# broadinstitute/Tangram

Hardware: NVIDIA H100
Metric: map_cells_to_space iterations/sec (higher is better)
Workload: dtype bf16 operands / f32 accumulate+state

## Files before the change

tangram_b200/csrc/gemm_tc.cuh:

```cuda
#pragma once
#include <cuda.h>
#include <cstdio>
#include "common.cuh"
#include "gemm_simt.cuh"

namespace tgb {

constexpr int TC_BM = 128;
constexpr int TC_BK = 64;
constexpr int TC_MMA_K = 16;
constexpr int TC_BN = 256;
constexpr int TC_THREADS = 384;
constexpr int TC_ACC = TC_BN / 2;

__device__ __forceinline__ uint32_t smem_u32(const void* p) { return (uint32_t)__cvta_generic_to_shared(p); }

__device__ __forceinline__ void mbar_init(uint64_t* bar, uint32_t count) {
  asm volatile("mbarrier.init.shared::cta.b64 [%0], %1;" ::"r"(smem_u32(bar)), "r"(count));
}
__device__ __forceinline__ void mbar_expect_tx(uint64_t* bar, uint32_t bytes) {
  asm volatile("mbarrier.arrive.expect_tx.shared::cta.b64 _, [%0], %1;" ::"r"(smem_u32(bar)), "r"(bytes) : "memory");
}
__device__ __forceinline__ void mbar_wait(uint64_t* bar, uint32_t parity) {
  asm volatile(
// ... 27 lines not shown
constexpr uint64_t kPolicyEvictLast = 0x14F0000000000000ull;
constexpr uint64_t kPolicyEvictFirst = 0x12F0000000000000ull;
__device__ __forceinline__ void prefetch_l2(const void* p) { asm volatile("prefetch.global.L2 [%0];" ::"l"(p)); }
__device__ __forceinline__ void tma_load_2d(const CUtensorMap* map, uint64_t* bar, void* dst, int c0, int c1, uint64_t policy) {
  asm volatile(
      "cp.async.bulk.tensor.2d.shared::cluster.global.tile.mbarrier::complete_tx::bytes.L2::cache_hint [%0], [%1, {%3, %4}], [%2], %5;"
      ::"r"(smem_u32(dst)), "l"(map), "r"(smem_u32(bar)), "r"(c0), "r"(c1), "l"(policy) : "memory");
}
__device__ __forceinline__ void tma_load_2d_pair(const CUtensorMap* map, uint64_t* bar, void* dst, int c0, int c1, uint64_t policy) {
  asm volatile(
      "cp.async.bulk.tensor.2d.shared::cluster.global.tile.mbarrier::complete_tx::bytes.multicast::cluster.L2::cache_hint"
      " [%0], [%1, {%3, %4}], [%2], %5, %6;"
      ::"r"(smem_u32(dst)), "l"(map), "r"(smem_u32(bar)), "r"(c0), "r"(c1), "h"((uint16_t)0x3), "l"(policy) : "memory");
}
__device__ __forceinline__ void tma_prefetch_desc(const CUtensorMap* map) {
  asm volatile("prefetch.tensormap [%0];" ::"l"(map) : "memory");
}
__device__ __forceinline__ void tma_store_2d(const CUtensorMap* map, const void* src, int c0, int c1, uint64_t policy) {
  asm volatile(
      "cp.async.bulk.tensor.2d.global.shared::cta.bulk_group.L2::cache_hint [%0, {%2, %3}], [%1], %4;"
      ::"l"(map), "r"(smem_u32(src)), "r"(c0), "r"(c1), "l"(policy) : "memory");
}
__device__ __forceinline__ void bulk_commit() { asm volatile("cp.async.bulk.commit_group;" ::: "memory"); }
__device__ __forceinline__ void bulk_wait_read_all() { asm volatile("cp.async.bulk.wait_group.read 0;" ::: "memory"); }
__device__ __forceinline__ void fence_proxy_async_smem() { asm volatile("fence.proxy.async.shared::cta;" ::: "memory"); }
template <int ID>
__device__ __forceinline__ void named_bar_sync(int threads) {
  asm volatile("bar.sync %0, %1;" ::"n"(ID), "r"(threads) : "memory");
}
__device__ __forceinline__ void ldmatrix_x4(uint32_t addr, uint32_t (&r)[4]) {
  asm volatile("ldmatrix.sync.aligned.m8n8.x4.shared.b16 {%0, %1, %2, %3}, [%4];"
               : "=r"(r[0]), "=r"(r[1]), "=r"(r[2]), "=r"(r[3]) : "r"(addr) : "memory");
}
__device__ __forceinline__ void stmatrix_x4(uint32_t addr, const uint32_t (&r)[4]) {
  asm volatile("stmatrix.sync.aligned.m8n8.x4.shared.b16 [%0], {%1, %2, %3, %4};"
               ::"r"(addr), "r"(r[0]), "r"(r[1]), "r"(r[2]), "r"(r[3]) : "memory");
}

__device__ __forceinline__ void setmaxnreg_producer() { asm volatile("setmaxnreg.dec.sync.aligned.u32 40;"); }
__device__ __forceinline__ void setmaxnreg_consumer() { asm volatile("setmaxnreg.inc.sync.aligned.u32 232;"); }

__device__ __forceinline__ void wgmma_fence() { asm volatile("wgmma.fence.sync.aligned;" ::: "memory"); }
__device__ __forceinline__ void wgmma_commit() { asm volatile("wgmma.commit_group.sync.aligned;" ::: "memory"); }
template <int N>
__device__ __forceinline__ void wgmma_wait() { asm volatile("wgmma.wait_group.sync.aligned %0;" ::"n"(N) : "memory"); }
__device__ __forceinline__ void acc_fence(float (&d)[TC_ACC]) {
#pragma unroll
  for (int i = 0; i < TC_ACC; ++i) asm volatile("" : "+f"(d[i])::"memory");
}

template <int TA, int TB>
__device__ __forceinline__ void wgmma_m64n256k16(float (&d)[128], uint64_t a_desc, uint64_t b_desc, uint32_t accumulate) {
  asm volatile(
      "{\n\t.reg .pred p;\n\t"
      "setp.ne.b32 p, %130, 0;\n\t"
      "wgmma.mma_async.sync.aligned.m64n256k16.f32.bf16.bf16 {"
      "%0,%1,%2,%3,%4,%5,%6,%7,%8,%9,%10,%11,%12,%13,%14,%15,"
      "%16,%17,%18,%19,%20,%21,%22,%23,%24,%25,%26,%27,%28,%29,%30,%31,"
      "%32,%33,%34,%35,%36,%37,%38,%39,%40,%41,%42,%43,%44,%45,%46,%47,"
      "%48,%49,%50,%51,%52,%53,%54,%55,%56,%57,%58,%59,%60,%61,%62,%63,"
      "%64,%65,%66,%67,%68,%69,%70,%71,%72,%73,%74,%75,%76,%77,%78,%79,"
      "%80,%81,%82,%83,%84,%85,%86,%87,%88,%89,%90,%91,%92,%93,%94,%95,"
      "%96,%97,%98,%99,%100,%101,%102,%103,%104,%105,%106,%107,%108,%109,%110,%111,"
      "%112,%113,%114,%115,%116,%117,%118,%119,%120,%121,%122,%123,%124,%125,%126,%127"
      "}, %128, %129, p, 1, 1, %131, %132;\n\t}"
      : "+f"(d[0]), "+f"(d[1]), "+f"(d[2]), "+f"(d[3]), "+f"(d[4]), "+f"(d[5]), "+f"(d[6]), "+f"(d[7]),
        "+f"(d[8]), "+f"(d[9]), "+f"(d[10]), "+f"(d[11]), "+f"(d[12]), "+f"(d[13]), "+f"(d[14]), "+f"(d[15]),
        "+f"(d[16]), "+f"(d[17]), "+f"(d[18]), "+f"(d[19]), "+f"(d[20]), "+f"(d[21]), "+f"(d[22]), "+f"(d[23]),
        "+f"(d[24]), "+f"(d[25]), "+f"(d[26]), "+f"(d[27]), "+f"(d[28]), "+f"(d[29]), "+f"(d[30]), "+f"(d[31]),
        "+f"(d[32]), "+f"(d[33]), "+f"(d[34]), "+f"(d[35]), "+f"(d[36]), "+f"(d[37]), "+f"(d[38]), "+f"(d[39]),
        "+f"(d[40]), "+f"(d[41]), "+f"(d[42]), "+f"(d[43]), "+f"(d[44]), "+f"(d[45]), "+f"(d[46]), "+f"(d[47]),
        "+f"(d[48]), "+f"(d[49]), "+f"(d[50]), "+f"(d[51]), "+f"(d[52]), "+f"(d[53]), "+f"(d[54]), "+f"(d[55]),
        "+f"(d[56]), "+f"(d[57]), "+f"(d[58]), "+f"(d[59]), "+f"(d[60]), "+f"(d[61]), "+f"(d[62]), "+f"(d[63]),
        "+f"(d[64]), "+f"(d[65]), "+f"(d[66]), "+f"(d[67]), "+f"(d[68]), "+f"(d[69]), "+f"(d[70]), "+f"(d[71]),
        "+f"(d[72]), "+f"(d[73]), "+f"(d[74]), "+f"(d[75]), "+f"(d[76]), "+f"(d[77]), "+f"(d[78]), "+f"(d[79]),
        "+f"(d[80]), "+f"(d[81]), "+f"(d[82]), "+f"(d[83]), "+f"(d[84]), "+f"(d[85]), "+f"(d[86]), "+f"(d[87]),
        "+f"(d[88]), "+f"(d[89]), "+f"(d[90]), "+f"(d[91]), "+f"(d[92]), "+f"(d[93]), "+f"(d[94]), "+f"(d[95]),
        "+f"(d[96]), "+f"(d[97]), "+f"(d[98]), "+f"(d[99]), "+f"(d[100]), "+f"(d[101]), "+f"(d[102]), "+f"(d[103]),
        "+f"(d[104]), "+f"(d[105]), "+f"(d[106]), "+f"(d[107]), "+f"(d[108]), "+f"(d[109]), "+f"(d[110]), "+f"(d[111]),
        "+f"(d[112]), "+f"(d[113]), "+f"(d[114]), "+f"(d[115]), "+f"(d[116]), "+f"(d[117]), "+f"(d[118]), "+f"(d[119]),
        "+f"(d[120]), "+f"(d[121]), "+f"(d[122]), "+f"(d[123]), "+f"(d[124]), "+f"(d[125]), "+f"(d[126]), "+f"(d[127])
      : "l"(a_desc), "l"(b_desc), "r"(accumulate), "n"(TA), "n"(TB));
}
__device__ __forceinline__ uint64_t make_smem_desc(uint32_t saddr, uint32_t lbo_bytes, uint32_t sbo_bytes) {
  uint64_t d = 0;
  d |= (uint64_t)((saddr & 0x3FFFF) >> 4);
  d |= (uint64_t)((lbo_bytes >> 4) & 0x3FFF) << 16;
  d |= (uint64_t)((sbo_bytes >> 4) & 0x3FFF) << 32;
  d |= (uint64_t)1 << 62;
  return d;
}

template <bool KMAJOR, int ROWS>
struct OperandTile {
  static constexpr int kBytes = ROWS * TC_BK * 2;
  static __device__ __forceinline__ void load(const CUtensorMap* map, uint64_t* bar, uint8_t* dst, int mn0, int k0, uint64_t policy) {
    if (KMAJOR) {
      tma_load_2d(map, bar, dst, k0, mn0, policy);
    } else {
#pragma unroll
      for (int b = 0; b < ROWS / 64; ++b) tma_load_2d(map, bar, dst + b * 8192, mn0 + b * 64, k0, policy);
    }
  }
  static __device__ __forceinline__ void load_half_pair(const CUtensorMap* map, uint64_t* bar, uint8_t* dst, int mn0, int k0, int h,
                                                        uint64_t policy) {
    constexpr int HALF = ROWS / 2;
    if (KMAJOR) {
      tma_load_2d_pair(map, bar, dst + h * HALF * 128, k0, mn0 + h * HALF, policy);
    } else {
#pragma unroll
      for (int b = 0; b < HALF / 64; ++b)
        tma_load_2d_pair(map, bar, dst + h * HALF * 128 + b * 8192, mn0 + h * HALF + b * 64, k0, policy);
    }
  }
  static __device__ __forceinline__ uint64_t desc(uint32_t saddr, int k_step ) {
    if (KMAJOR) return make_smem_desc(saddr + k_step * (TC_MMA_K * 2), 16, 1024);
    return make_smem_desc(saddr + k_step * (TC_MMA_K * 128), 8192, 1024);
  }
};

struct EpiSmem {
  uint8_t* buf;
  uint64_t* full;
  uint64_t* free;
  uint32_t parity;
};
__device__ __forceinline__ void tile_mn(int w, int tiles_m, int tiles_n, int group_m, int& m, int& n) {
  const int per_group = group_m * tiles_n;
  const int g = w / per_group, r = w - g * per_group;
  const int rows = min(group_m, tiles_m - g * group_m);
  n = r / rows;
  m = g * group_m + (r - n * rows);
}
struct TileCoord {
  int m0, n0;
  int tile_n;
  int tiles_n;
  int split;
};

__device__ __forceinline__ float quad_sum(float v) {
  v += __shfl_xor_sync(0xffffffffu, v, 1);
  v += __shfl_xor_sync(0xffffffffu, v, 2);
  return v;
}

struct TcEpiStore {
  static constexpr int kSmemBytes = 0;
  float* C; int ldc; size_t split_stride; int M;
  int accumulate;
  __device__ __forceinline__ void prologue(const TileCoord&, int) const {}
  __device__ __forceinline__ void load(int, int, const EpiSmem&) const {}
  __device__ __forceinline__ void run(const float (&d)[TC_ACC], const TileCoord& t, int row, int lane, int, const EpiSmem&) const {
    float* base = C + (size_t)t.split * split_stride;
#pragma unroll
    for (int h = 0; h < 2; ++h) {
      const int r = row + 8 * h;
      if (r >= M) continue;
#pragma unroll
      for (int j = 0; j < TC_BN / 8; ++j) {
        const int col = t.n0 + 8 * j + 2 * (lane & 3);
        if (col < ldc) {
          float2* dst = reinterpret_cast<float2*>(base + (size_t)r * ldc + col);
          float2 v = make_float2(d[4 * j + 2 * h], d[4 * j + 2 * h + 1]);
          if (accumulate) { const float2 o = *dst; v.x += o.x; v.y += o.y; }
          *dst = v;
        }
      }
    }
  }
};

struct TcEpiDpStore {
  static constexpr int kSmemBytes = TC_BM * TC_BN * 2;
  static constexpr int kHalfBytes = kSmemBytes / 2;
  static constexpr int kBoxBytes = 64 * 128;
  CUtensorMap pt_map, dq_map;
  int ld;
  const float* center;
  float* rpart;
  int M;
  __device__ __forceinline__ int boxes(int r0, int n0) const { return r0 < M ? min(TC_BN / 64, (ld - n0) / 64) : 0; }
  __device__ __forceinline__ void prologue(const TileCoord&, int) const {}
  __device__ __forceinline__ void load(int m0, int n0, const EpiSmem& es) const {
#pragma unroll
    for (int h = 0; h < 2; ++h) {
      mbar_wait(&es.free[h], es.parity ^ 1);
      const int nb = boxes(m0 + 64 * h, n0);
      mbar_expect_tx(&es.full[h], nb * kBoxBytes);
      for (int b = 0; b < nb; ++b)
        tma_load_2d(&pt_map, &es.full[h], es.buf + h * kHalfBytes + b * kBoxBytes, n0 + 64 * b, m0 + 64 * h, kPolicyEvictFirst);
    }
  }
  __device__ __forceinline__ void run(const float (&d)[TC_ACC], const TileCoord& t, int row, int lane, int cw,
                                      const EpiSmem& es) const {
    const int r0 = t.m0 + 64 * cw;
    const int nb = boxes(r0, t.n0);
    float c[2];
#pragma unroll
    for (int h = 0; h < 2; ++h) c[h] = row + 8 * h < M ? center[row + 8 * h] : 0.f;
    const int mi = lane >> 3, rr = lane & 7;
    const int arow = ((row - r0) & ~15) + 8 * (mi & 1) + rr;
    const uint32_t half = smem_u32(es.buf + cw * kHalfBytes) + arow * 128;
    mbar_wait(&es.full[cw], es.parity);
    float racc[2] = {0.f, 0.f};
#pragma unroll
    for (int b = 0; b < TC_BN / 64; ++b) {
      if (b >= nb) break;
#pragma unroll
      for (int q = 0; q < 4; ++q) {
        const uint32_t addr = half + b * kBoxBytes + (((2 * q + (mi >> 1)) ^ rr) << 4);
        uint32_t p[4], o[4];
        ldmatrix_x4(addr, p);
#pragma unroll
        for (int e = 0; e < 2; ++e) {
          const int j = 8 * b + 2 * q + e;
#pragma unroll
          for (int h = 0; h < 2; ++h) {
            const __nv_bfloat162 d2 = __floats2bfloat162_rn(d[4 * j + 2 * h] - c[h], d[4 * j + 2 * h + 1] - c[h]);
            const __nv_bfloat162 p2 = *reinterpret_cast<const __nv_bfloat162*>(&p[2 * e + h]);
            racc[h] = fmaf(__low2float(p2), __low2float(d2), racc[h]);
            racc[h] = fmaf(__high2float(p2), __high2float(d2), racc[h]);
            o[2 * e + h] = *reinterpret_cast<const uint32_t*>(&d2);
          }
        }
        stmatrix_x4(addr, o);
      }
    }
    fence_proxy_async_smem();
    if (cw == 0) named_bar_sync<1>(128); else named_bar_sync<2>(128);
    if ((threadIdx.x & 127) == 0) {
      for (int b = 0; b < nb; ++b) tma_store_2d(&dq_map, es.buf + cw * kHalfBytes + b * kBoxBytes, t.n0 + 64 * b, r0, kPolicyEvictFirst);
      bulk_commit();
      bulk_wait_read_all();
      mbar_arrive(&es.free[cw]);
    }
#pragma unroll
    for (int h = 0; h < 2; ++h) {
      const float s = quad_sum(racc[h]);
      if (row + 8 * h < M && (lane & 3) == 0) rpart[(size_t)t.tile_n * M + row + 8 * h] = s;
    }
  }
};

struct TcEpiDpStoreF32 {
  static constexpr int kSmemBytes = 0;
  float* dp; int ld;
  const __nv_bfloat16* P3; size_t plane;
  float* rpart;
  int M;
  __device__ __forceinline__ void prologue(const TileCoord& t, int ct) const {
#pragma unroll
    for (int i = ct; i < 3 * TC_BM * (TC_BN / 64); i += 256) {
      const int pl = i / (TC_BM * (TC_BN / 64)), li = i - pl * (TC_BM * (TC_BN / 64));
      const int row = t.m0 + (li >> 2), col = t.n0 + (li & 3) * 64;
      if (row < M && col < ld) prefetch_l2(P3 + pl * plane + (size_t)row * ld + col);
    }
  }
  __device__ __forceinline__ void load(int, int, const EpiSmem&) const {}
  __device__ __forceinline__ void run(const float (&d)[TC_ACC], const TileCoord& t, int row, int lane, int, const EpiSmem&) const {
#pragma unroll
    for (int h = 0; h < 2; ++h) {
      const int r = row + 8 * h;
      const bool live = r < M;
      const __nv_bfloat16* prow = P3 + (size_t)r * ld;
      float* drow = dp + (size_t)r * ld;
      float racc = 0.f;
#pragma unroll
      for (int j = 0; j < TC_BN / 8; ++j) {
        const int col = t.n0 + 8 * j + 2 * (lane & 3);
        if (live && col < ld) {
          const __nv_bfloat162 h2 = *reinterpret_cast<const __nv_bfloat162*>(prow + col);
          const __nv_bfloat162 m2 = *reinterpret_cast<const __nv_bfloat162*>(prow + plane + col);
          const __nv_bfloat162 l2 = *reinterpret_cast<const __nv_bfloat162*>(prow + 2 * plane + col);
          const float p0 = (__low2float(l2) + __low2float(m2)) + __low2float(h2);
          const float p1 = (__high2float(l2) + __high2float(m2)) + __high2float(h2);
          const float v0 = d[4 * j + 2 * h], v1 = d[4 * j + 2 * h + 1];
          racc = fmaf(p0, v0, racc);
          racc = fmaf(p1, v1, racc);
          *reinterpret_cast<float2*>(drow + col) = make_float2(v0, v1);
        }
      }
      racc = quad_sum(racc);
      if (live && (lane & 3) == 0) rpart[(size_t)t.tile_n * M + r] = racc;
    }
  }
};

struct __align__(16) RowConst { float lse, r, h, pad; };

__device__ __forceinline__ float fast_ex2(float x) { float y; asm("ex2.approx.ftz.f32 %0, %1;" : "=f"(y) : "f"(x)); return y; }
__device__ __forceinline__ float fast_rcp(float x) { float y; asm("rcp.approx.ftz.f32 %0, %1;" : "=f"(y) : "f"(x)); return y; }
__device__ __forceinline__ float fast_sqrt(float x) { float y; asm("sqrt.approx.ftz.f32 %0, %1;" : "=f"(y) : "f"(x)); return y; }

struct TcMaps { CUtensorMap m[3]; };
__device__ __constant__ int kPairA[6] = {2, 0, 1, 1, 0, 0};
__device__ __constant__ int kPairB[6] = {0, 2, 1, 0, 1, 0};

template <bool A_KMAJOR, bool B_KMAJOR, int STAGES, class Epi>
__global__ void __launch_bounds__(TC_THREADS, 1)
k_gemm_tc(const __grid_constant__ TcMaps maps_a, const __grid_constant__ TcMaps maps_b, int n_pairs,
          int k_total, int k_per_split, int tiles_m, int tiles_n, int splits, int group_m, uint64_t policy_a,
          uint64_t policy_b, int tm_off, int k_off, const __grid_constant__ Epi epi) {
  using TileA = OperandTile<A_KMAJOR, TC_BM>;
  using TileB = OperandTile<B_KMAJOR, TC_BN>;
  constexpr int kStageBytes = TileA::kBytes + TileB::kBytes;
  constexpr int kTA = A_KMAJOR ? 0 : 1, kTB = B_KMAJOR ? 0 : 1;
  constexpr uint32_t kConsumerWarps = 8;

  extern __shared__ uint8_t smem_raw[];
  uint8_t* smem = reinterpret_cast<uint8_t*>(((uintptr_t)smem_raw + 1023) & ~(uintptr_t)1023);
  __shared__ __align__(8) uint64_t full_bar[STAGES];
  __shared__ __align__(8) uint64_t empty_bar[STAGES];
  __shared__ __align__(8) uint64_t epi_full[2], epi_free[2];

  const int wg = threadIdx.x >> 7, lane = threadIdx.x & 31;
  const int tiles_mp = (tiles_m + 1) / 2;
  const int total = tiles_mp * tiles_n * splits;
  EpiSmem es{smem + STAGES * kStageBytes, epi_full, epi_free, 0};

  if (threadIdx.x == 0) {
    tma_prefetch_desc(&maps_a.m[0]);
    tma_prefetch_desc(&maps_b.m[0]);
#pragma unroll
    for (int s = 0; s < STAGES; ++s) { mbar_init(&full_bar[s], 1); mbar_init(&empty_bar[s], 2 * kConsumerWarps); }
    if constexpr (Epi::kSmemBytes > 0) {
      for (int h = 0; h < 2; ++h) { mbar_init(&epi_full[h], 1); mbar_init(&epi_free[h], 1); }
    }
    fence_barrier_init();
  }
  cluster_sync();

  if (wg == 0) {
    setmaxnreg_producer();
    if (threadIdx.x == 0) {
      uint32_t kbg = 0;
      for (int w = cluster_index(); w < total; w += cluster_count()) {
        const int z = w / (tiles_n * tiles_mp);
        int tp_i, tn_i;
        tile_mn(w - z * tiles_n * tiles_mp, tiles_mp, tiles_n, group_m, tp_i, tn_i);
        const int tm_i = 2 * tp_i + cluster_rank();
        const bool live = tm_i < tiles_m;
        const int n0 = tn_i * TC_BN, m0 = (tm_off + tm_i) * TC_BM;
        const int k_begin = k_off + z * k_per_split;
        const int k_end = min(k_total, k_begin + k_per_split);
        const int num_kb = (k_end - k_begin + TC_BK - 1) / TC_BK;
        for (int pr = 6 - n_pairs; pr < 6; ++pr) {
          const CUtensorMap* ma = &maps_a.m[kPairA[pr]];
          const CUtensorMap* mb = &maps_b.m[kPairB[pr]];
#pragma unroll 1
          for (int kb = 0; kb < num_kb; ++kb, ++kbg) {
            const int s = kbg % STAGES;
            const uint32_t ph = (kbg / STAGES) & 1;
            mbar_wait(&empty_bar[s], ph ^ 1);
            uint8_t* sa = smem + s * kStageBytes;
            uint8_t* sb = sa + TileA::kBytes;
            mbar_expect_tx(&full_bar[s], live ? kStageBytes : TileB::kBytes);
            const int k0 = k_begin + kb * TC_BK;
            if (live) TileA::load(ma, &full_bar[s], sa, m0, k0, policy_a);
            TileB::load_half_pair(mb, &full_bar[s], sb, n0, k0, cluster_rank(), policy_b);
#ifndef TGB_SKIP_EPI
            if (Epi::kSmemBytes > 0 && live && pr == 6 - n_pairs && kb + 1 == min(STAGES, num_kb)) epi.load(m0, n0, es);
#endif
          }
        }
        if (live) es.parity ^= 1;
      }
    }
  } else {
    setmaxnreg_consumer();
    const int cw = wg - 1;
    const int ct = threadIdx.x - 128;
    const int row_in_tile = 64 * cw + 16 * ((threadIdx.x >> 5) & 3) + (lane >> 2);
    float acc[TC_ACC];
#pragma unroll
    for (int i = 0; i < TC_ACC; ++i) acc[i] = 0.f;
    uint32_t kbg = 0;
    for (int w = cluster_index(); w < total; w += cluster_count()) {
      TileCoord t;
      t.split = w / (tiles_n * tiles_mp);
      int tp_i;
      tile_mn(w - t.split * tiles_n * tiles_mp, tiles_mp, tiles_n, group_m, tp_i, t.tile_n);
      t.tiles_n = tiles_n;
      t.n0 = t.tile_n * TC_BN;
      t.m0 = (tm_off + 2 * tp_i + cluster_rank()) * TC_BM;
      const bool live = t.m0 < (tm_off + tiles_m) * TC_BM;
      const int k_begin = k_off + t.split * k_per_split;
      const int k_end = min(k_total, k_begin + k_per_split);
      const int total_kb = (k_end - k_begin + TC_BK - 1) / TC_BK * n_pairs;
#ifndef TGB_SKIP_EPI
      if (live) epi.prologue(t, ct);
#endif
      acc_fence(acc);
      for (int kb = 0; kb < total_kb; ++kb, ++kbg) {
        const int s = kbg % STAGES;
        const uint32_t ph = (kbg / STAGES) & 1;
        mbar_wait(&full_bar[s], ph);
        const uint32_t sa = smem_u32(smem + s * kStageBytes) + cw * 8192;
        const uint32_t sb = smem_u32(smem + s * kStageBytes) + TileA::kBytes;
        wgmma_fence();
#pragma unroll
        for (int k = 0; k < TC_BK / TC_MMA_K; ++k)
          wgmma_m64n256k16<kTA, kTB>(acc, TileA::desc(sa, k), TileB::desc(sb, k), (kb > 0 || k > 0) ? 1u : 0u);
        wgmma_commit();
        wgmma_wait<1>();
        if (kb > 0 && lane < 2) mbar_arrive_cluster(&empty_bar[(kbg - 1) % STAGES], lane);
      }
      wgmma_wait<0>();
      acc_fence(acc);
      if (total_kb > 0 && lane < 2) mbar_arrive_cluster(&empty_bar[(kbg - 1) % STAGES], lane);
#ifndef TGB_SKIP_EPI
      if (t.m0 < (tm_off + tiles_m) * TC_BM) {
        epi.run(acc, t, t.m0 + row_in_tile, lane, cw, es);
        es.parity ^= 1;
      }
#endif
    }
  }
  cluster_sync();
}

typedef CUresult (*PFN_encodeTiled)(CUtensorMap*, CUtensorMapDataType, cuuint32_t, void*, const cuuint64_t*,
                                    const cuuint64_t*, const cuuint32_t*, const cuuint32_t*, CUtensorMapInterleave,
                                    CUtensorMapSwizzle, CUtensorMapL2promotion, CUtensorMapFloatOOBfill);

struct TcContext {
  PFN_encodeTiled encode = nullptr;
  int num_sms = 132;
  const void* smem_fn[16] = {};
  int smem_bytes[16] = {};
  int clusters[16] = {};
};

static inline int tc_init(TcContext& tc, char* err, size_t n) {
  void* fn = nullptr;
  cudaDriverEntryPointQueryResult qres;
  cudaError_t e = cudaGetDriverEntryPoint("cuTensorMapEncodeTiled", &fn, cudaEnableDefault, &qres);
  if (e != cudaSuccess || fn == nullptr || qres != cudaDriverEntryPointSuccess) {
    snprintf(err, n, "cuTensorMapEncodeTiled not available from the driver (%s)", cudaGetErrorString(e));
    return -2;
  }
  tc.encode = (PFN_encodeTiled)fn;
  int dev = 0;
  cudaGetDevice(&dev);
  cudaDeviceGetAttribute(&tc.num_sms, cudaDevAttrMultiProcessorCount, dev);
  return 0;
}

static inline int tc_make_map(TcContext& tc, CUtensorMap* map, const void* base, uint64_t cols, uint64_t rows,
                              uint64_t ld, uint32_t box_inner, uint32_t box_outer, char* err, size_t n) {
// ... 153 lines not shown
```

tangram_b200/csrc/tangram_b200.cu:

```cuda
#include "../../include/tangram_b200.h"

#include <algorithm>
#include <cmath>
#include <cstdarg>
#include <cstdio>
#include <cstdlib>
#include <cstring>
#include <mutex>
#include <string>
#include <thread>
#include <vector>

#include "common.cuh"
#include "kernels_elem.cuh"
#include "gemm_simt.cuh"
#include "gemm_tc.cuh"
#include "adam_rows.cuh"
#include "legacy_rng.cuh"
#include "agreement.cuh"
#include "annotate.cuh"
#include "project.cuh"
#include "group_stats.cuh"
#include "neighbors.cuh"
#include "mt19937_jump.h"
// ... 2718 lines not shown
  }
  int bad_host = 0;
  CK(cudaMemcpyAsync(&bad_host, bad.p, sizeof(int), cudaMemcpyDeviceToHost, s));
  CK(cudaStreamSynchronize(s));
  if (bad_host)
    return fail(TGB200_ERR_INVALID, "a CSR column index is outside [0, %lld) or not strictly increasing within its row",
                (long long)n_genes);
  CK(cudaMemcpyAsync(sum_out, sum.p, sizeof(double) * T * G, cudaMemcpyDefault, s));
  CK(cudaMemcpyAsync(sumsq_out, sq.p, sizeof(double) * T * G, cudaMemcpyDefault, s));
  if (nnz_out) CK(cudaMemcpyAsync(nnz_out, cntd.p, sizeof(int64_t) * T * G, cudaMemcpyDefault, s));
  CK(cudaStreamSynchronize(s));
  return TGB200_OK;
}

extern "C" int tgb200_group_stats(const float* X, int64_t x_ld, const int64_t* indptr, const int32_t* indices,
                                  const float* data, int64_t nnz, int64_t rows, int64_t n_genes,
                                  const int32_t* labels, int32_t n_labels, double* sum_out, double* sumsq_out,
                                  int64_t* nnz_out, int64_t block_rows, int32_t device, void* stream) {
  return group_stats_pass(GsValue::kIdentity, 1.0, X, x_ld, indptr, indices, data, nnz, rows, n_genes, labels, n_labels,
                          sum_out, sumsq_out, nnz_out, block_rows, device, stream);
}

extern "C" int tgb200_group_stats_expm1(const float* X, int64_t x_ld, const int64_t* indptr, const int32_t* indices,
                                        const float* data, int64_t nnz, int64_t rows, int64_t n_genes,
                                        const int32_t* labels, int32_t n_labels, double* sum_out, double* sumsq_out,
                                        int64_t* nnz_out, int64_t block_rows, int32_t device, void* stream,
                                        double scale) {
  if (!std::isfinite(scale)) return fail(TGB200_ERR_INVALID, "scale=%g is not finite", scale);
  return group_stats_pass(GsValue::kExpm1, scale, X, x_ld, indptr, indices, data, nnz, rows, n_genes, labels, n_labels,
                          sum_out, sumsq_out, nnz_out, block_rows, device, stream);
}

#ifdef TGB_OVERLAP_PROBE
extern "C" TGB200_API int tgb200_debug_overlap_probe(tgb200_mapper* h, int32_t kind, int32_t cap, int32_t update_ctas,
                                                     int32_t what, int32_t reps, float* out) {
  if (!h || !out || reps < 1 || what < 1 || what > 3) return fail(TGB200_ERR_INVALID, "bad argument");
  if (!h->bf16 || !h->pipelined || h->host_state || !h->plan_dp.ready || !h->plan_fwd.ready)
    return fail(TGB200_ERR_STATE, "needs a resident, pipelined bf16 handle that has run an iteration");
  CK(cudaSetDevice(h->cfg.device));
  const int c0 = h->chunk_row[0], c1 = h->chunk_row[1], c2 = h->chunk_row[2];
  const AdamScalars a = adam_scalars(h->cfg, h->step > 0 ? h->step : 1, 0.1f);
  const AdamRowsArgs ar{h->M.p, h->mb.p, h->v.p, h->dq.p, h->Pb.p, reinterpret_cast<const RowConst*>(h->rowc.p),
                        h->zsum.p, h->pxsum.p, h->l1sum.p, h->l2sum.p, h->ld, h->V, c0, c1,
                        h->cfg.lambda_r, h->cfg.lambda_l1, h->cfg.lambda_l2, a};
  const bool plain = ar.lam_r == 0.f && ar.lam_l1 == 0.f && ar.lam_l2 == 0.f;
  const int keep = cap > 0 ? std::max(0, h->tc.num_sms - 2 * cap) : 0;
  cudaEvent_t ev[4];
  for (auto& e : ev) CK(cudaEventCreate(&e));
  int st = TGB200_OK;
  CK(cudaDeviceSynchronize());
  for (int r = 0; r < reps && st == TGB200_OK; ++r) {
    CK(cudaEventRecord(ev[0], h->hi));
    CK(cudaStreamWaitEvent(h->lo, ev[0], 0));
    if (what & 1) {
      if (kind == 0) {
        TcEpiDpStore epi{h->plan_dp.pt, h->plan_dp.dq, h->ld, h->rcenter.p, h->rpart.p, h->N};
        st = tc_dpstore_launch(h->tc, h->plan_dp, 1, epi, c1, c2, h->V, h->Ke, keep, h->hi, g_err, sizeof(g_err));
      } else {
        st = tc_forward_launch_rows(h->tc, h->plan_fwd, 1, h->Y.p, 1, c1, c2, h->V, h->Ke, keep, h->hi, g_err, sizeof(g_err));
      }
    }
    if (what & 2) {
      if (update_ctas <= 0) {
        if (adam_rows_launch(ar, h->lo)) st = fail(TGB200_ERR_CUDA, "launch adam_rows");
      } else if (plain) {
        k_adam_rows_probe<true><<<update_ctas, 512, 0, h->lo>>>(ar);
      } else {
        k_adam_rows_probe<false><<<update_ctas, 512, 0, h->lo>>>(ar);
      }
      if (cudaGetLastError() != cudaSuccess) st = fail(TGB200_ERR_CUDA, "launch adam_rows_probe");
    }
    CK(cudaEventRecord(ev[1], h->hi));
    CK(cudaEventRecord(ev[2], h->lo));
    CK(cudaStreamWaitEvent(h->hi, ev[2], 0));
    CK(cudaEventRecord(ev[3], h->hi));
    CK(cudaEventSynchronize(ev[3]));
    for (int i = 0; i < 3; ++i) CK(cudaEventElapsedTime(&out[3 * r + i], ev[0], ev[i + 1]));
  }
  for (auto& e : ev) cudaEventDestroy(e);
  return st;
}
#endif

namespace {
constexpr int64_t kNbMaxCellsPerAxis = int64_t(1) << 24;
constexpr int64_t kNbMaxCells = int64_t(1) << 28;

int64_t nb_cell_cap(int64_t n) { return std::min<int64_t>(2 * n + 64, kNbMaxCells); }

nb::Grid nb_grid(const double lo[3], const double ext[3], int64_t n, double per_cell, double min_h, int64_t cap) {
  double log_vol = 0.0, max_ext = 0.0;
  int d_eff = 0;
  for (int a = 0; a < 3; ++a) {
    if (ext[a] > 0) { log_vol += std::log(ext[a]); ++d_eff; }
    max_ext = std::max(max_ext, ext[a]);
  }
  double h = d_eff ? std::exp((log_vol + std::log(per_cell / (double)n)) / d_eff) : 1.0;
  h = std::max(h, min_h);
  if (!(h > 0) || !std::isfinite(1.0 / h)) h = max_ext > 0 ? max_ext : 1.0;
  nb::Grid g{};
  for (;;) {
    const double inv = 1.0 / h;
    double total = 1.0;
    bool ok = true;
    for (int a = 0; a < 3; ++a) {
      const double c = std::floor(ext[a] * inv) + 1.0;
      ok &= c <= (double)kNbMaxCellsPerAxis;
      total *= c;
    }
    if (ok && total <= (double)cap) {
      g.inv_h = inv;
      for (int a = 0; a < 3; ++a) { g.lo[a] = lo[a]; g.nc[a] = (int)(std::floor(ext[a] * inv) + 1.0); }
      break;
    }
    h *= 1.25;
  }
  g.h_lo = (1.0 / g.inv_h) * (1.0 - 1e-9);
  if (!(g.h_lo > 1e-150)) g.h_lo = 0.0;
  return g;
}

struct NbSearch {
  DevBuf<double> C, xs, ys, zs;
  DevBuf<int> orig, cell, count, bad;
  DevBuf<long long> start, tiles;
  DevBuf<unsigned long long> box;
  nb::Grid g{};
  int n = 0;
  nb::Points points() const { return nb::Points{xs.p, ys.p, zs.p, orig.p, start.p}; }
};

int64_t nb_scan_tiles(int64_t n) { return ceil_div(n, nb::kScanTile); }

int nb_scan(const int* in, int64_t n, long long* out, long long* tiles, cudaStream_t s) {
  const int64_t nt = nb_scan_tiles(n);
  nb::k_nb_scan_tiles<<<(unsigned)nt, 256, 0, s>>>(in, n, out, tiles);
  CK(cudaGetLastError());
  lrng::k_scan_counts<<<1, 1024, 0, s>>>(tiles, (int)nt, tiles + nt + 1);
  CK(cudaGetLastError());
  nb::k_nb_scan_add<<<(unsigned)ceil_div(n + 1, nb::kThreads), nb::kThreads, 0, s>>>(out, n, tiles + nt + 1, (int)nt);
  CK(cudaGetLastError());
  return TGB200_OK;
}

double nb_search_bytes(int64_t n, int dim) {
  const int64_t cells = nb_cell_cap(n);
  return 8.0 * n * dim + 32.0 * n + 4.0 * n + 12.0 * (cells + 1) + 16.0 * (nb_scan_tiles(std::max(cells, n) + 1) + 1);
}

int nb_build(const double* coords, int64_t n, int dim, double per_cell, double min_h, double out_bytes, int32_t device,
             cudaStream_t s, const char* what, NbSearch& S) {
  int n_sms = 0;
  CKS(use_sm90_device(device, &n_sms));
  size_t free_b = 0, total_b = 0;
  CK(cudaMemGetInfo(&free_b, &total_b));
  const double need = nb_search_bytes(n, dim) + out_bytes, avail = (double)free_b - 256.0 * (1 << 20);
  if (need > avail)
    return fail(TGB200_ERR_INVALID, "%s over %lld points in %d-D needs %.3f GiB on device %d (%.3f GiB of it for the "
                "output); %.3f GiB are free", what, (long long)n, dim, need / 1073741824.0, device,
                out_bytes / 1073741824.0, free_b / 1073741824.0);
  S.n = (int)n;
  CKS(S.C.alloc((size_t)n * dim, false));
  CK(cudaMemcpyAsync(S.C.p, coords, sizeof(double) * n * dim, cudaMemcpyDefault, s));
  unsigned long long box0[6];
  for (int a = 0; a < 3; ++a) { box0[2 * a] = ~0ull; box0[2 * a + 1] = 0ull; }
  CKS(S.box.alloc(6, false));
// ... 118 lines not shown
```

Measured before the change: 48.08.

## Defer dP-store epilogue into next tile's mainloop to overlap with wgmma

The DpStore epilogue becomes deferred. Each consumer packs its accumulator into bf16 registers and spreads the ldmatrix/stmatrix, TMA store and row-reduction work for the previous tile across specific k-blocks of the next tile's mainloop. The P-tile smem buffer is halved and loaded in two rounds by the producer at chosen k-blocks. A first-MMA variant that zeroes the accumulator replaces explicit accumulator reuse. An optional compile-time phase probe is also added. This aims to hide the epilogue latency behind tensor-core work, at the cost of extra registers (64 packed words) and more complex barrier/parity bookkeeping.

```diff
diff --git a/tangram_b200/csrc/gemm_tc.cuh b/tangram_b200/csrc/gemm_tc.cuh
--- a/tangram_b200/csrc/gemm_tc.cuh
+++ b/tangram_b200/csrc/gemm_tc.cuh
@@ -133,6 +133,39 @@
         "+f"(d[120]), "+f"(d[121]), "+f"(d[122]), "+f"(d[123]), "+f"(d[124]), "+f"(d[125]), "+f"(d[126]), "+f"(d[127])
       : "l"(a_desc), "l"(b_desc), "r"(accumulate), "n"(TA), "n"(TB));
 }
+template <int TA, int TB>
+__device__ __forceinline__ void wgmma_m64n256k16_first(float (&d)[128], uint64_t a_desc, uint64_t b_desc) {
+  asm volatile(
+      "{\n\t.reg .pred p;\n\t"
+      "setp.ne.b32 p, 0, 0;\n\t"
+      "wgmma.mma_async.sync.aligned.m64n256k16.f32.bf16.bf16 {"
+      "%0,%1,%2,%3,%4,%5,%6,%7,%8,%9,%10,%11,%12,%13,%14,%15,"
+      "%16,%17,%18,%19,%20,%21,%22,%23,%24,%25,%26,%27,%28,%29,%30,%31,"
+      "%32,%33,%34,%35,%36,%37,%38,%39,%40,%41,%42,%43,%44,%45,%46,%47,"
+      "%48,%49,%50,%51,%52,%53,%54,%55,%56,%57,%58,%59,%60,%61,%62,%63,"
+      "%64,%65,%66,%67,%68,%69,%70,%71,%72,%73,%74,%75,%76,%77,%78,%79,"
+      "%80,%81,%82,%83,%84,%85,%86,%87,%88,%89,%90,%91,%92,%93,%94,%95,"
+      "%96,%97,%98,%99,%100,%101,%102,%103,%104,%105,%106,%107,%108,%109,%110,%111,"
+      "%112,%113,%114,%115,%116,%117,%118,%119,%120,%121,%122,%123,%124,%125,%126,%127"
+      "}, %128, %129, p, 1, 1, %130, %131;\n\t}"
+      : "=f"(d[0]), "=f"(d[1]), "=f"(d[2]), "=f"(d[3]), "=f"(d[4]), "=f"(d[5]), "=f"(d[6]), "=f"(d[7]),
+        "=f"(d[8]), "=f"(d[9]), "=f"(d[10]), "=f"(d[11]), "=f"(d[12]), "=f"(d[13]), "=f"(d[14]), "=f"(d[15]),
+        "=f"(d[16]), "=f"(d[17]), "=f"(d[18]), "=f"(d[19]), "=f"(d[20]), "=f"(d[21]), "=f"(d[22]), "=f"(d[23]),
+        "=f"(d[24]), "=f"(d[25]), "=f"(d[26]), "=f"(d[27]), "=f"(d[28]), "=f"(d[29]), "=f"(d[30]), "=f"(d[31]),
+        "=f"(d[32]), "=f"(d[33]), "=f"(d[34]), "=f"(d[35]), "=f"(d[36]), "=f"(d[37]), "=f"(d[38]), "=f"(d[39]),
+        "=f"(d[40]), "=f"(d[41]), "=f"(d[42]), "=f"(d[43]), "=f"(d[44]), "=f"(d[45]), "=f"(d[46]), "=f"(d[47]),
+        "=f"(d[48]), "=f"(d[49]), "=f"(d[50]), "=f"(d[51]), "=f"(d[52]), "=f"(d[53]), "=f"(d[54]), "=f"(d[55]),
+        "=f"(d[56]), "=f"(d[57]), "=f"(d[58]), "=f"(d[59]), "=f"(d[60]), "=f"(d[61]), "=f"(d[62]), "=f"(d[63]),
+        "=f"(d[64]), "=f"(d[65]), "=f"(d[66]), "=f"(d[67]), "=f"(d[68]), "=f"(d[69]), "=f"(d[70]), "=f"(d[71]),
+        "=f"(d[72]), "=f"(d[73]), "=f"(d[74]), "=f"(d[75]), "=f"(d[76]), "=f"(d[77]), "=f"(d[78]), "=f"(d[79]),
+        "=f"(d[80]), "=f"(d[81]), "=f"(d[82]), "=f"(d[83]), "=f"(d[84]), "=f"(d[85]), "=f"(d[86]), "=f"(d[87]),
+        "=f"(d[88]), "=f"(d[89]), "=f"(d[90]), "=f"(d[91]), "=f"(d[92]), "=f"(d[93]), "=f"(d[94]), "=f"(d[95]),
+        "=f"(d[96]), "=f"(d[97]), "=f"(d[98]), "=f"(d[99]), "=f"(d[100]), "=f"(d[101]), "=f"(d[102]), "=f"(d[103]),
+        "=f"(d[104]), "=f"(d[105]), "=f"(d[106]), "=f"(d[107]), "=f"(d[108]), "=f"(d[109]), "=f"(d[110]), "=f"(d[111]),
+        "=f"(d[112]), "=f"(d[113]), "=f"(d[114]), "=f"(d[115]), "=f"(d[116]), "=f"(d[117]), "=f"(d[118]), "=f"(d[119]),
+        "=f"(d[120]), "=f"(d[121]), "=f"(d[122]), "=f"(d[123]), "=f"(d[124]), "=f"(d[125]), "=f"(d[126]), "=f"(d[127])
+      : "l"(a_desc), "l"(b_desc), "n"(TA), "n"(TB));
+}
 __device__ __forceinline__ uint64_t make_smem_desc(uint32_t saddr, uint32_t lbo_bytes, uint32_t sbo_bytes) {
   uint64_t d = 0;
   d |= (uint64_t)((saddr & 0x3FFFF) >> 4);
@@ -169,6 +202,27 @@
     return make_smem_desc(saddr + k_step * (TC_MMA_K * 128), 8192, 1024);
   }
 };
+
+#ifdef TGB_BWD_PHASE_PROBE
+enum { kBwdProbeFull, kBwdProbeRetired, kBwdProbePtFull, kBwdProbeStmatrix, kBwdProbeStore, kBwdProbeRead, kBwdProbeSm, kBwdProbeNs };
+__device__ unsigned long long* g_bwd_probe;
+__device__ __forceinline__ void bwd_probe(long long tile, int cw, int what) {
+  if (g_bwd_probe == nullptr || tile < 0 || (threadIdx.x & 127) != 0) return;
+  unsigned long long* p = g_bwd_probe + (tile * 2 + cw) * 8;
+  p[what] = clock64();
+  if (what == kBwdProbeFull) {
+    unsigned long long ns;
+    uint32_t sm;
+    asm volatile("mov.u64 %0, %%globaltimer;" : "=l"(ns));
+    asm volatile("mov.u32 %0, %%smid;" : "=r"(sm));
+    p[kBwdProbeSm] = sm;
+    p[kBwdProbeNs] = ns;
+  }
+}
+#define TGB_BWD_PROBE(tile, cw, what) bwd_probe(tile, cw, what)
+#else
+#define TGB_BWD_PROBE(tile, cw, what) ((void)0)
+#endif
 
 struct EpiSmem {
   uint8_t* buf;
@@ -198,6 +252,7 @@
 
 struct TcEpiStore {
   static constexpr int kSmemBytes = 0;
+  static constexpr bool kDeferred = false;
   float* C; int ldc; size_t split_stride; int M;
   int accumulate;
   __device__ __forceinline__ void prologue(const TileCoord&, int) const {}
@@ -223,79 +278,115 @@
 };
 
 struct TcEpiDpStore {
-  static constexpr int kSmemBytes = TC_BM * TC_BN * 2;
+  static constexpr int kSmemBytes = TC_BM * (TC_BN / 2) * 2;
   static constexpr int kHalfBytes = kSmemBytes / 2;
   static constexpr int kBoxBytes = 64 * 128;
+  static constexpr bool kDeferred = true;
+  static constexpr int kSteps = 8;
+  static constexpr int kRound1Kb = 10;
+  static __host__ __device__ constexpr int step_kb(int s) { return s < 4 ? s : kRound1Kb + s - 4; }
+  static constexpr int kLoadKb1 = 8, kLoadKb0 = 18;
   CUtensorMap pt_map, dq_map;
   int ld;
   const float* center;
   float* rpart;
   int M;
   __device__ __forceinline__ int boxes(int r0, int n0) const { return r0 < M ? min(TC_BN / 64, (ld - n0) / 64) : 0; }
-  __device__ __forceinline__ void prologue(const TileCoord&, int) const {}
-  __device__ __forceinline__ void load(int m0, int n0, const EpiSmem& es) const {
+  __device__ __forceinline__ long long tile_id(int m0, int tile_n) const { return (long long)(m0 / TC_BM) * ((ld + TC_BN - 1) / TC_BN) + tile_n; }
+  __device__ __forceinline__ void centres(int row, float (&c)[2]) const {
+#pragma unroll
+    for (int h = 0; h < 2; ++h) c[h] = row + 8 * h < M ? center[row + 8 * h] : 0.f;
+  }
+  static __device__ __forceinline__ void pack(const float (&d)[TC_ACC], const float (&c)[2], uint32_t (&v)[TC_ACC / 2]) {
+#pragma unroll
+    for (int j = 0; j < TC_BN / 8; ++j) {
+#pragma unroll
+      for (int h = 0; h < 2; ++h) {
+        const __nv_bfloat162 d2 = __floats2bfloat162_rn(d[4 * j + 2 * h] - c[h], d[4 * j + 2 * h + 1] - c[h]);
+        v[2 * j + h] = *reinterpret_cast<const uint32_t*>(&d2);
+      }
+    }
+  }
+  __device__ __forceinline__ void step(int s, const uint32_t (&v)[TC_ACC / 2], float (&racc)[2], int m0, int tile_n, int row,
+                                       int lane, int cw, EpiSmem& es) const {
+    const int r0 = m0 + 64 * cw, n0 = tile_n * TC_BN;
+    const int nb = boxes(r0, n0);
+    const int round = s / 4, sr = s % 4;
+    if (sr < 2) {
+      const int b = 2 * round + sr;
+      const int mi = lane >> 3, rr = lane & 7;
+      const int arow = ((row - r0) & ~15) + 8 * (mi & 1) + rr;
+      const uint32_t half = smem_u32(es.buf + cw * kHalfBytes) + arow * 128;
+      if (sr == 0) {
+        mbar_wait(&es.full[cw], es.parity);
+        if (round == 0) {
+          TGB_BWD_PROBE(tile_id(m0, tile_n), cw, kBwdProbePtFull);
+          racc[0] = racc[1] = 0.f;
+        }
+      }
+      if (b < nb) {
+#pragma unroll
+        for (int q = 0; q < 4; ++q) {
+          const uint32_t addr = half + sr * kBoxBytes + (((2 * q + (mi >> 1)) ^ rr) << 4);
+          uint32_t p[4], o[4];
+          ldmatrix_x4(addr, p);
+#pragma unroll
+          for (int e = 0; e < 2; ++e) {
+            const int j = 8 * b + 2 * q + e;
+#pragma unroll
+            for (int h = 0; h < 2; ++h) {
+              const __nv_bfloat162 d2 = *reinterpret_cast<const __nv_bfloat162*>(&v[2 * j + h]);
+              const __nv_bfloat162 p2 = *reinterpret_cast<const __nv_bfloat162*>(&p[2 * e + h]);
+              racc[h] = fmaf(__low2float(p2), __low2float(d2), racc[h]);
+              racc[h] = fmaf(__high2float(p2), __high2float(d2), racc[h]);
+              o[2 * e + h] = v[2 * j + h];
+            }
+          }
+          stmatrix_x4(addr, o);
+        }
+      }
+      if (b == TC_BN / 64 - 1) TGB_BWD_PROBE(tile_id(m0, tile_n), cw, kBwdProbeStmatrix);
+    } else if (sr == 2) {
+      fence_proxy_async_smem();
+      if (cw == 0) named_bar_sync<1>(128); else named_bar_sync<2>(128);
+      if ((threadIdx.x & 127) == 0) {
+        for (int b = 2 * round; b < min(nb, 2 * round + 2); ++b)
+          tma_store_2d(&dq_map, es.buf + cw * kHalfBytes + (b - 2 * round) * kBoxBytes, n0 + 64 * b, r0, kPolicyEvictFirst);
+        bulk_commit();
+      }
+      if (round == 1) {
+        TGB_BWD_PROBE(tile_id(m0, tile_n), cw, kBwdProbeStore);
+#pragma unroll
+        for (int h = 0; h < 2; ++h) {
+          const float sum = quad_sum(racc[h]);
+          if (row + 8 * h < M && (lane & 3) == 0) rpart[(size_t)tile_n * M + row + 8 * h] = sum;
+        }
+      }
+    } else {
+      if ((threadIdx.x & 127) == 0) {
+        bulk_wait_read_all();
+        if (round == 1) TGB_BWD_PROBE(tile_id(m0, tile_n), cw, kBwdProbeRead);
+        mbar_arrive(&es.free[cw]);
+      }
+      es.parity ^= 1;
+    }
+  }
+  __device__ __forceinline__ void load(int m0, int n0, int r, const EpiSmem& es) const {
 #pragma unroll
     for (int h = 0; h < 2; ++h) {
       mbar_wait(&es.free[h], es.parity ^ 1);
-      const int nb = boxes(m0 + 64 * h, n0);
+      const int nb = min(2, max(0, boxes(m0 + 64 * h, n0) - 2 * r));
       mbar_expect_tx(&es.full[h], nb * kBoxBytes);
       for (int b = 0; b < nb; ++b)
-        tma_load_2d(&pt_map, &es.full[h], es.buf + h * kHalfBytes + b * kBoxBytes, n0 + 64 * b, m0 + 64 * h, kPolicyEvictFirst);
-    }
-  }
-  __device__ __forceinline__ void run(const float (&d)[TC_ACC], const TileCoord& t, int row, int lane, int cw,
-                                      const EpiSmem& es) const {
-    const int r0 = t.m0 + 64 * cw;
-    const int nb = boxes(r0, t.n0);
-    float c[2];
-#pragma unroll
-    for (int h = 0; h < 2; ++h) c[h] = row + 8 * h < M ? center[row + 8 * h] : 0.f;
-    const int mi = lane >> 3, rr = lane & 7;
-    const int arow = ((row - r0) & ~15) + 8 * (mi & 1) + rr;
-    const uint32_t half = smem_u32(es.buf + cw * kHalfBytes) + arow * 128;
-    mbar_wait(&es.full[cw], es.parity);
-    float racc[2] = {0.f, 0.f};
-#pragma unroll
-    for (int b = 0; b < TC_BN / 64; ++b) {
-      if (b >= nb) break;
-#pragma unroll
-      for (int q = 0; q < 4; ++q) {
-        const uint32_t addr = half + b * kBoxBytes + (((2 * q + (mi >> 1)) ^ rr) << 4);
-        uint32_t p[4], o[4];
-        ldmatrix_x4(addr, p);
-#pragma unroll
-        for (int e = 0; e < 2; ++e) {
-          const int j = 8 * b + 2 * q + e;
-#pragma unroll
-          for (int h = 0; h < 2; ++h) {
-            const __nv_bfloat162 d2 = __floats2bfloat162_rn(d[4 * j + 2 * h] - c[h], d[4 * j + 2 * h + 1] - c[h]);
-            const __nv_bfloat162 p2 = *reinterpret_cast<const __nv_bfloat162*>(&p[2 * e + h]);
-            racc[h] = fmaf(__low2float(p2), __low2float(d2), racc[h]);
-            racc[h] = fmaf(__high2float(p2), __high2float(d2), racc[h]);
-            o[2 * e + h] = *reinterpret_cast<const uint32_t*>(&d2);
-          }
-        }
-        stmatrix_x4(addr, o);
-      }
-    }
-    fence_proxy_async_smem();
-    if (cw == 0) named_bar_sync<1>(128); else named_bar_sync<2>(128);
-    if ((threadIdx.x & 127) == 0) {
-      for (int b = 0; b < nb; ++b) tma_store_2d(&dq_map, es.buf + cw * kHalfBytes + b * kBoxBytes, t.n0 + 64 * b, r0, kPolicyEvictFirst);
-      bulk_commit();
-      bulk_wait_read_all();
-      mbar_arrive(&es.free[cw]);
-    }
-#pragma unroll
-    for (int h = 0; h < 2; ++h) {
-      const float s = quad_sum(racc[h]);
-      if (row + 8 * h < M && (lane & 3) == 0) rpart[(size_t)t.tile_n * M + row + 8 * h] = s;
+        tma_load_2d(&pt_map, &es.full[h], es.buf + h * kHalfBytes + b * kBoxBytes, n0 + 128 * r + 64 * b, m0 + 64 * h,
+                    kPolicyEvictFirst);
     }
   }
 };
 
 struct TcEpiDpStoreF32 {
   static constexpr int kSmemBytes = 0;
+  static constexpr bool kDeferred = false;
   float* dp; int ld;
   const __nv_bfloat16* P3; size_t plane;
   float* rpart;
@@ -386,6 +477,8 @@
     setmaxnreg_producer();
     if (threadIdx.x == 0) {
       uint32_t kbg = 0;
+      int prev_m0 = -1, prev_n0 = 0;
+      (void)prev_n0;
       for (int w = cluster_index(); w < total; w += cluster_count()) {
         const int z = w / (tiles_n * tiles_mp);
         int tp_i, tn_i;
@@ -411,12 +504,95 @@
             if (live) TileA::load(ma, &full_bar[s], sa, m0, k0, policy_a);
             TileB::load_half_pair(mb, &full_bar[s], sb, n0, k0, cluster_rank(), policy_b);
 #ifndef TGB_SKIP_EPI
-            if (Epi::kSmemBytes > 0 && live && pr == 6 - n_pairs && kb + 1 == min(STAGES, num_kb)) epi.load(m0, n0, es);
+            if constexpr (Epi::kSmemBytes > 0) {
+              if (pr == 6 - n_pairs) {
+                if (prev_m0 >= 0 && kb + 1 == min(Epi::kLoadKb1, num_kb)) {
+                  epi.load(prev_m0, prev_n0, 1, es);
+                  es.parity ^= 1;
+                  prev_m0 = -1;
+                }
+                if (live && kb + 1 == min(Epi::kLoadKb0, num_kb)) {
+                  epi.load(m0, n0, 0, es);
+                  es.parity ^= 1;
+                }
+              }
+            }
 #endif
           }
         }
-        if (live) es.parity ^= 1;
-      }
+        if (live) { prev_m0 = m0; prev_n0 = n0; }
+      }
+#ifndef TGB_SKIP_EPI
+      if constexpr (Epi::kSmemBytes > 0) {
+        if (prev_m0 >= 0) epi.load(prev_m0, prev_n0, 1, es);
+      }
+#endif
+    }
+  } else if constexpr (Epi::kDeferred) {
+    setmaxnreg_consumer();
+    const int cw = wg - 1;
+    const int row_in_tile = 64 * cw + 16 * ((threadIdx.x >> 5) & 3) + (lane >> 2);
+    float acc[TC_ACC];
+#pragma unroll
+    for (int i = 0; i < TC_ACC; ++i) acc[i] = 0.f;
+    uint32_t dq[TC_ACC / 2];
+    float racc[2] = {0.f, 0.f};
+    int pend_m0 = -1, pend_tn = 0;
+    uint32_t kbg = 0;
+    auto kblock = [&](int kb, long long probe_tile) {
+      const int s = kbg % STAGES;
+      const uint32_t ph = (kbg / STAGES) & 1;
+      mbar_wait(&full_bar[s], ph);
+      if (kb == 0) TGB_BWD_PROBE(probe_tile, cw, kBwdProbeFull);
+      const uint32_t sa = smem_u32(smem + s * kStageBytes) + cw * 8192;
+      const uint32_t sb = smem_u32(smem + s * kStageBytes) + TileA::kBytes;
+      wgmma_fence();
+#pragma unroll
+      for (int k = 0; k < TC_BK / TC_MMA_K; ++k) {
+        if (kb == 0 && k == 0) wgmma_m64n256k16_first<kTA, kTB>(acc, TileA::desc(sa, k), TileB::desc(sb, k));
+        else wgmma_m64n256k16<kTA, kTB>(acc, TileA::desc(sa, k), TileB::desc(sb, k), 1u);
+      }
+      wgmma_commit();
+      wgmma_wait<1>();
+      if (kb > 0 && lane < 2) mbar_arrive_cluster(&empty_bar[(kbg - 1) % STAGES], lane);
+      ++kbg;
+    };
+    for (int w = cluster_index(); w < total; w += cluster_count()) {
+      const int split = w / (tiles_n * tiles_mp);
+      int tp_i, tile_n;
+      tile_mn(w - split * tiles_n * tiles_mp, tiles_mp, tiles_n, group_m, tp_i, tile_n);
+      const int m0 = (tm_off + 2 * tp_i + cluster_rank()) * TC_BM;
+      const bool live = m0 < (tm_off + tiles_m) * TC_BM;
+      const int k_begin = k_off + split * k_per_split;
+      const int k_end = min(k_total, k_begin + k_per_split);
+      const int total_kb = (k_end - k_begin + TC_BK - 1) / TC_BK * n_pairs;
+      const long long probe_tile = live ? epi.tile_id(m0, tile_n) : -1;
+      (void)probe_tile;
+      float c[2] = {0.f, 0.f};
+      if (live) epi.centres(m0 + row_in_tile, c);
+      acc_fence(acc);
+      constexpr int kPrefix = Epi::step_kb(Epi::kSteps - 1) + 1;
+#pragma unroll
+      for (int p = 0; p < kPrefix; ++p) {
+        if (p == 0 || p < total_kb) kblock(p, probe_tile);
+#pragma unroll
+        for (int s = 0; s < Epi::kSteps; ++s)
+          if (Epi::step_kb(s) == p && pend_m0 >= 0) epi.step(s, dq, racc, pend_m0, pend_tn, pend_m0 + row_in_tile, lane, cw, es);
+      }
+      for (int kb = kPrefix; kb < total_kb; ++kb) kblock(kb, probe_tile);
+      wgmma_wait<0>();
+      acc_fence(acc);
+      if (live) TGB_BWD_PROBE(probe_tile, cw, kBwdProbeRetired);
+      if (total_kb > 0 && lane < 2) mbar_arrive_cluster(&empty_bar[(kbg - 1) % STAGES], lane);
+#ifndef TGB_SKIP_EPI
+      Epi::pack(acc, c, dq);
+      pend_m0 = live ? m0 : -1;
+      pend_tn = tile_n;
+#endif
+    }
+    if (pend_m0 >= 0) {
+#pragma unroll
+      for (int s = 0; s < Epi::kSteps; ++s) epi.step(s, dq, racc, pend_m0, pend_tn, pend_m0 + row_in_tile, lane, cw, es);
     }
   } else {
     setmaxnreg_consumer();
diff --git a/tangram_b200/csrc/tangram_b200.cu b/tangram_b200/csrc/tangram_b200.cu
--- a/tangram_b200/csrc/tangram_b200.cu
+++ b/tangram_b200/csrc/tangram_b200.cu
@@ -2824,6 +2824,16 @@
 }
 #endif
 
+#ifdef TGB_BWD_PHASE_PROBE
+extern "C" TGB200_API int tgb200_debug_bwd_phase_probe(tgb200_mapper* h, void* buf) {
+  if (!h) return fail(TGB200_ERR_INVALID, "bad argument");
+  CK(cudaSetDevice(h->cfg.device));
+  CK(cudaDeviceSynchronize());
+  CK(cudaMemcpyToSymbol(g_bwd_probe, &buf, sizeof(buf)));
+  return TGB200_OK;
+}
+#endif
+
 namespace {
 constexpr int64_t kNbMaxCellsPerAxis = int64_t(1) << 24;
 constexpr int64_t kNbMaxCells = int64_t(1) << 28;
```

New measurement: 50.18 (median of 6 runs). +4.4%, better.
